# mpt0816/Cilqr

Hardware: AMD Instinct MI355X
Metric: CILQR solves/sec (50-step horizon, batch=65536 per GPU) (higher is better)
Workload: dtype f64

## Files before the change

### cilqr_amd/csrc/cost_reduce.hpp

```cpp
#pragma once
#include "dev_model.hpp"
#include "ref_order.hpp"

namespace cilqr {

CILQR_DEV void reduce_cost(const DeviceState& s, int slot, int cand, double* c5) {
#ifdef CILQR_REF_ORDER
  const int buf = s.cur[slot] ^ cand;
  reforder::total_cost(
      s, slot, [&](int i, double* x) { load_x(s, buf, i, slot, x); }, [&](int i, double* u) { load_u(s, buf, i, slot, u); }, c5);
#else
  (void)cand;
  const int Bc = s.Bcap, K = s.p.K, N = s.p.N;
  double j = 0.0, dx = 0.0, du = 0.0, cc = 0.0, lc = 0.0;
#pragma unroll 8
  for (int i = 0; i < K; ++i) {
    const double2* o = s.part + (size_t)i * kPartPairs * Bc + slot;
    const double2 a = o[0], c = o[(size_t)2 * Bc];
    j += a.x;
    dx += a.y;
    cc += c.x;
    lc += c.y;
  }
#pragma unroll 8
  for (int i = 0; i < N; ++i) {
    const double2 b = s.part[((size_t)i * kPartPairs + 1) * Bc + slot];
    j += b.x;
    du += b.y;
  }
  const double dyn = dx + du;
  c5[0] = j + dyn + cc + lc;
  c5[1] = j; c5[2] = dyn; c5[3] = cc; c5[4] = lc;
#endif
}

#ifdef CILQR_REF_ORDER
CILQR_DEV void spec_total_cost(const DeviceState& s, int slot, int r, int j, double* c5) {
  const size_t cap = (size_t)s.spec_cap;
  reforder::total_cost(
      s, slot,
      [&](int i, double* x) {
        const double2* xb = s.Xs + ((size_t)r * s.p.K + i) * 3 * cap + j;
        const double2 p0 = xb[0], p1 = xb[cap], p2 = xb[2 * cap];
        x[0] = p0.x; x[1] = p0.y; x[2] = p1.x; x[3] = p1.y; x[4] = p2.x; x[5] = p2.y;
      },
      [&](int i, double* u) {
        const double2 q = s.Us[((size_t)r * s.p.N + i) * cap + j];
        u[0] = q.x; u[1] = q.y;
      },
      c5);
}
#endif

}
```

### cilqr_amd/csrc/kernels_quad.hip

```cpp
#include "quad_core.hpp"

namespace cilqr {

#ifndef CILQR_COST_OCC
#define CILQR_COST_OCC 4
#endif
#define CILQR_COST_ATTR __attribute__((amdgpu_waves_per_eu(CILQR_COST_OCC, CILQR_COST_OCC)))
#define CILQR_LAUNCH_BY_DISCS(kernel, grid, block, lds, st, ...)                                            \
  do {                                                                                                     \
    if (s.p.num_of_disc == 5) {                                                                            \
      if (s.exact_ties) hipLaunchKernelGGL((kernel<5, true>), grid, block, lds, st, __VA_ARGS__);          \
      else hipLaunchKernelGGL((kernel<5, false>), grid, block, lds, st, __VA_ARGS__);                      \
    } else {                                                                                               \
      if (s.exact_ties) hipLaunchKernelGGL((kernel<0, true>), grid, block, lds, st, __VA_ARGS__);          \
      else hipLaunchKernelGGL((kernel<0, false>), grid, block, lds, st, __VA_ARGS__);                      \
    }                                                                                                      \
  } while (0)

template <int D, bool EX>
__global__ __launch_bounds__(256) CILQR_COST_ATTR void k_cost_knots(DeviceState s, const int* __restrict__ list,
                                                    const int* __restrict__ n_ptr, int n_max, int cand,
                                                    int skip_done) {
  extern __shared__ double lds[];
#ifdef CILQR_COST_PROFILE
  unsigned long long cp_t = wall_clock64();
  const unsigned long long cp_t0 = cp_t;
#endif
  const int n = n_ptr ? min(*n_ptr, n_max) : active_count(s, n_max);
  if ((int)(blockIdx.x * blockDim.x) >= n) return;
  const double* lanes = stage_lanes(s, lds);
  CP_STAMP(0);
  const int i = blockIdx.y;
// ... 21 lines not shown
#ifdef CILQR_COST_PROFILE
extern "C" void cilqr_debug_cost_profile(unsigned long long* out, int reset) {
  if (out) (void)hipMemcpyFromSymbol(out, HIP_SYMBOL(g_cost_prof), sizeof(g_cost_prof));
  if (reset) { void* p = nullptr; (void)hipGetSymbolAddress(&p, HIP_SYMBOL(g_cost_prof)); (void)hipMemset(p, 0, sizeof(g_cost_prof)); }
}
#endif

template <int D, bool EX>
__global__ __launch_bounds__(256) CILQR_COST_ATTR void k_spec_cost(DeviceState s, const int* __restrict__ list,
                                                   const int* __restrict__ n_ptr, int off, int n_max, int r0) {
  extern __shared__ double lds[];
  const int n = list_count(s, n_ptr, off, n_max);
  if ((int)(blockIdx.x * blockDim.x) >= n) return;
  const double* lanes = stage_lanes(s, lds);
  const int i = blockIdx.y, r = r0 + blockIdx.z;
  const size_t cap = (size_t)s.spec_cap;
  for (int j = blockIdx.x * blockDim.x + threadIdx.x; j < n; j += gridDim.x * blockDim.x) {
    const int slot = list[j];
    if (s.acc_idx[slot] != -1) continue;
    const double2* xb = s.Xs + ((size_t)r * s.p.K + i) * 3 * cap + j;
    const double2 p0 = xb[0], p1 = xb[cap], p2 = xb[2 * cap];
    const double x[6] = {p0.x, p0.y, p1.x, p1.y, p2.x, p2.y};
    double u[2] = {0.0, 0.0};
    if (i < s.p.N) {
      const double2 q = s.Us[((size_t)r * s.p.N + i) * cap + j];
      u[0] = q.x; u[1] = q.y;
    }
    knot_cost<D, EX>(s, lanes, i, slot, x, u, s.parts + ((size_t)r * s.p.K + i) * kPartPairs * cap + j, cap);
  }
}
template <int D, int P, bool EX>
__global__ __launch_bounds__(256) CILQR_COST_ATTR void k_spec_cost_packed(DeviceState s, const int* __restrict__ list,
                                                                          const int* __restrict__ n_ptr, int off, int n_max,
                                                                          int r0, int r_end) {
  extern __shared__ double lds[];
  const int n = list_count(s, n_ptr, off, n_max);
  constexpr int per_block = 256 / P;
  if ((int)(blockIdx.x * per_block) >= n) return;
  const double* lanes = stage_lanes(s, lds);
  const int i = blockIdx.y, r = r0 + (int)(threadIdx.x % P);
  const size_t cap = (size_t)s.spec_cap;
  if (r >= r_end) return;
  for (int j = blockIdx.x * per_block + threadIdx.x / P; j < n; j += gridDim.x * per_block) {
    const int slot = list[j];
    if (s.acc_idx[slot] != -1) continue;
    const double2* xb = s.Xs + ((size_t)r * s.p.K + i) * 3 * cap + j;
    const double2 p0 = xb[0], p1 = xb[cap], p2 = xb[2 * cap];
    const double x[6] = {p0.x, p0.y, p1.x, p1.y, p2.x, p2.y};
    double u[2] = {0.0, 0.0};
    if (i < s.p.N) {
      const double2 q = s.Us[((size_t)r * s.p.N + i) * cap + j];
      u[0] = q.x; u[1] = q.y;
    }
    knot_cost<D, EX>(s, lanes, i, slot, x, u, s.parts + ((size_t)r * s.p.K + i) * kPartPairs * cap + j, cap);
  }
}

void launch_spec_cost(const DeviceState& s, const int* list, const int* n_ptr, int off, int n_max, int n_grid, int r0,
                      int sparse, hipStream_t st) {
  const size_t lds = lane_lds_bytes(s);
  const bool five = s.p.num_of_disc == 5;
  if (!sparse) {
    dim3 g((n_grid + 255) / 256, s.p.K, kNumAlpha - r0);
    CILQR_LAUNCH_BY_DISCS(k_spec_cost, g, dim3(256), lds, st, s, list, n_ptr, off, n_max, r0);
    return;
  }
  for (int a = r0; a < kNumAlpha;) {
    const int left = kNumAlpha - a;
    const int P = left > 4 ? 8 : (left > 2 ? 4 : (left > 1 ? 2 : 1));
    const int e = a + (P < left ? P : left);
    const int per_block = 256 / P;
    dim3 g((n_grid + per_block - 1) / per_block, s.p.K);
#define CILQR_SC1(DD, PP, EE) hipLaunchKernelGGL((k_spec_cost_packed<DD, PP, EE>), g, dim3(256), lds, st, s, list, n_ptr, off, n_max, a, e)
#define CILQR_SC(DD, PP) do { if (s.exact_ties) CILQR_SC1(DD, PP, true); else CILQR_SC1(DD, PP, false); } while (0)
    if (P == 8) { if (five) CILQR_SC(5, 8); else CILQR_SC(0, 8); }
    else if (P == 4) { if (five) CILQR_SC(5, 4); else CILQR_SC(0, 4); }
    else if (P == 2) { if (five) CILQR_SC(5, 2); else CILQR_SC(0, 2); }
    else { if (five) CILQR_SC(5, 1); else CILQR_SC(0, 1); }
#undef CILQR_SC1
#undef CILQR_SC
    a = e;
  }
}

template <int D, int G, bool EX>
__global__ __launch_bounds__(256) CILQR_COST_ATTR void k_round_cost(DeviceState s, int r0, int n_max) {
  extern __shared__ double lds[];
  const int* __restrict__ list = s.pend + (size_t)r0 * s.Bcap;
  const int n = (r0 == 0) ? active_count(s, n_max) : min(s.counters[r0], n_max);
  constexpr int per_block = 256 / G;
  if ((int)(blockIdx.x * per_block) >= n) return;
  const double* lanes = stage_lanes(s, lds);
  const int i = blockIdx.y, r = r0 + (int)(threadIdx.x % G);
  const size_t cap = (size_t)s.spec_cap;
  for (int e = blockIdx.x * per_block + threadIdx.x / G; e < n; e += gridDim.x * per_block) {
    const int j = (r0 == 0) ? e : list[e];
    const int slot = s.act[j];
    if (s.acc_idx[slot] != -1) continue;
    const double2* xb = s.Xs + ((size_t)r * s.p.K + i) * 3 * cap + j;
    const double2 p0 = xb[0], p1 = xb[cap], p2 = xb[2 * cap];
    const double x[6] = {p0.x, p0.y, p1.x, p1.y, p2.x, p2.y};
    double u[2] = {0.0, 0.0};
    if (i < s.p.N) {
      const double2 q = s.Us[((size_t)r * s.p.N + i) * cap + j];
      u[0] = q.x; u[1] = q.y;
    }
    knot_cost<D, EX>(s, lanes, i, slot, x, u, s.parts + ((size_t)r * s.p.K + i) * kPartPairs * cap + j, cap);
  }
}

void launch_round_cost(const DeviceState& s, int r0, int group, int n_max, int n_grid, hipStream_t st) {
  const int per_block = 256 / group;
  dim3 g((n_grid + per_block - 1) / per_block, s.p.K);
  const size_t lds = lane_lds_bytes(s);
  const bool five = s.p.num_of_disc == 5;
#define CILQR_RC1(DD, GG, EE) hipLaunchKernelGGL((k_round_cost<DD, GG, EE>), g, dim3(256), lds, st, s, r0, n_max)
#define CILQR_RC(DD, GG) do { if (s.exact_ties) CILQR_RC1(DD, GG, true); else CILQR_RC1(DD, GG, false); } while (0)
  if (group == 1) { if (five) CILQR_RC(5, 1); else CILQR_RC(0, 1); }
  else if (group == 2) { if (five) CILQR_RC(5, 2); else CILQR_RC(0, 2); }
  else { if (five) CILQR_RC(5, 4); else CILQR_RC(0, 4); }
#undef CILQR_RC
#undef CILQR_RC1
}

__global__ __launch_bounds__(64) void k_reduce_only(DeviceState s, const int* __restrict__ list, int n) {
  const int j = blockIdx.x * blockDim.x + threadIdx.x;
  if (j >= n) return;
  const int slot = list ? list[j] : j;
  double c5[5];
  reduce_cost(s, slot, 0, c5);
#pragma unroll
  for (int c = 0; c < 5; ++c) s.trial[(size_t)c * s.Bcap + slot] = c5[c];
}

void launch_cost_knots(const DeviceState& s, const int* list, const int* n_ptr, int n_max, int n_grid,
                       int cand, int skip_done, hipStream_t st) {
  if (n_grid <= 0) return;
  dim3 g((n_grid + 255) / 256, s.p.K);
  CILQR_LAUNCH_BY_DISCS(k_cost_knots, g, dim3(256), lane_lds_bytes(s), st, s, list, n_ptr, n_max, cand, skip_done);
}

void launch_cost_only(const DeviceState& s, const int* list, int n, int cand, hipStream_t st) {
  if (n == 0) return;
  launch_cost_knots(s, list, nullptr, n, n, cand, 0, st);
  hipLaunchKernelGGL(k_reduce_only, dim3((n + 63) / 64), dim3(64), 0, st, s, list, n);
}

__global__ void k_init_cost_commit(DeviceState s, int n) {
  const int slot = blockIdx.x * blockDim.x + threadIdx.x;
// ... 51 lines not shown
```

### cilqr_amd/csrc/kernels_search.hip

```cpp
#include <cstdio>
#include <cstdlib>

#include "search_core.hpp"

namespace cilqr {

#ifndef CILQR_ROLL_OCC
#define CILQR_ROLL_OCC 0
#endif
#if CILQR_ROLL_OCC > 0
#define CILQR_ROLL_ATTR __attribute__((amdgpu_waves_per_eu(CILQR_ROLL_OCC, CILQR_ROLL_OCC)))
#else
#define CILQR_ROLL_ATTR
#endif
__global__ __launch_bounds__(64) CILQR_ROLL_ATTR void k_forward(DeviceState s, const int* __restrict__ list, int n,
                                                double alpha, int skip_done) {
  const int j = blockIdx.x * blockDim.x + threadIdx.x;
  if (j >= n) return;
  const int slot = list ? list[j] : j;
  if (skip_done && s.acc_idx[slot] != -1) return;
  forward_problem(s, slot, alpha);
}
void launch_forward(const DeviceState& s, const int* list, int n, double alpha, int skip_done,
                    hipStream_t st) {
// ... 43 lines not shown
                                                            const int* __restrict__ n_ptr, int off, int n_max, int r0) {
  const int n = list_count(s, n_ptr, off, n_max);
  constexpr int per_block = 64 / 8;
  const int r = r0 + (threadIdx.x & 7);
  if (r >= kNumAlpha) return;
  for (int j = blockIdx.x * per_block + threadIdx.x / 8; j < n; j += gridDim.x * per_block) {
    const int slot = list[j];
    forward_core(s, slot, kAlpha[r], OutSpec{s, r, j});
  }
}

__global__ __launch_bounds__(64) CILQR_ROLL_ATTR void k_spec_forward(DeviceState s, const int* __restrict__ list,
                                                     const int* __restrict__ n_ptr, int off, int n_max, int r0, int open) {
  const int n = list_count(s, n_ptr, off, n_max);
  const int r = r0 + blockIdx.y;
  for (int j = blockIdx.x * blockDim.x + threadIdx.x; j < n; j += gridDim.x * blockDim.x) {
    const int slot = list[j];
    if (open) {
      if (leaves_before_search(s, slot, r == 0)) {
        if (r == 0) s.acc_idx[slot] = -2;
        continue;
      }
      if (r == 0) s.acc_idx[slot] = -1;
    }
    forward_core(s, slot, kAlpha[r], OutSpec{s, r, j});
  }
}

__global__ __launch_bounds__(64) void k_spec_reduce(DeviceState s, const int* __restrict__ list,
                                                    const int* __restrict__ n_ptr, int off, int n_max, int r0, int open) {
  const int n = list_count(s, n_ptr, off, n_max);
  const int r = r0 + blockIdx.y;
  const size_t cap = (size_t)s.spec_cap;
  const int K = s.p.K, N = s.p.N;
  for (int j = blockIdx.x * blockDim.x + threadIdx.x; j < n; j += gridDim.x * blockDim.x) {
    const int slot = list[j];
    if (open) {
      if (s.acc_idx[slot] != -1) continue;
    }
    double* t = s.spec_tot + (size_t)r * 5 * cap + j;
#ifdef CILQR_REF_ORDER
    double c5[5];
    spec_total_cost(s, slot, r, j, c5);
    t[0] = c5[0];
    t[cap] = c5[1]; t[2 * cap] = c5[2]; t[3 * cap] = c5[3]; t[4 * cap] = c5[4];
    (void)K; (void)N;
#else
    double jj = 0.0, dx = 0.0, du = 0.0, cc = 0.0, lc = 0.0;
    const double2* pb = s.parts + (size_t)r * K * kPartPairs * cap + j;
#pragma unroll 8
    for (int i = 0; i < K; ++i) {
      const double2* o = pb + (size_t)i * kPartPairs * cap;
      const double2 a = o[0], c = o[2 * cap];
      jj += a.x;
      dx += a.y;
      cc += c.x;
      lc += c.y;
    }
#pragma unroll 8
    for (int i = 0; i < N; ++i) {
      const double2 b = pb[((size_t)i * kPartPairs + 1) * cap];
      jj += b.x;
      du += b.y;
    }
    const double dyn = dx + du;
    t[0] = jj + dyn + cc + lc;
    t[cap] = jj; t[2 * cap] = dyn; t[3 * cap] = cc; t[4 * cap] = lc;
#endif
  }
}

__global__ __launch_bounds__(64) void k_spec_pick(DeviceState s, const int* __restrict__ list,
                                                  const int* __restrict__ n_ptr, int off, int n_max, int r0) {
  const int n = list_count(s, n_ptr, off, n_max);
  const size_t cap = (size_t)s.spec_cap;
  const int Bc = s.Bcap;
  for (int j = blockIdx.x * blockDim.x + threadIdx.x; j < n; j += gridDim.x * blockDim.x) {
    const int slot = list[j];
    if (s.acc_idx[slot] != -1) continue;
    const double cost_old = s.cost_old[slot], dV0 = s.dV[slot], dV1 = s.dV[(size_t)Bc + slot];
    int acc = -1, last = kNumAlpha - 1;
    double dcost = 0.0;
    double tot[kNumAlpha];
#pragma unroll
    for (int r = 0; r < kNumAlpha; ++r) tot[r] = (r >= r0) ? s.spec_tot[(size_t)r * 5 * cap + j] : 0.0;
#pragma unroll
    for (int r = 0; r < kNumAlpha; ++r) {
      if (r < r0) continue;
      const double alpha = kAlpha[r];
      dcost = cost_old - tot[r];
      const double expected = -alpha * (dV0 + alpha * dV1);
      const double z = dcost / expected;
      if ((z > 1e-4 && z < 10.0) && dcost > 0.0) {
        acc = r;
        last = r;
        break;
      }
    }
#pragma unroll
    for (int c = 0; c < 5; ++c)
      s.trial[(size_t)c * Bc + slot] = s.spec_tot[((size_t)last * 5 + c) * cap + j];
// ... 31 lines not shown
#ifndef CILQR_FWD_AHEAD
#define CILQR_FWD_AHEAD 1
#endif
template <int P>
__global__ __launch_bounds__(64) __attribute__((amdgpu_waves_per_eu(CILQR_FWD_OCC, CILQR_FWD_OCC)))
void k_multi_forward_packed(DeviceState s, int n, int G) {
  const int t = blockIdx.x * blockDim.x + threadIdx.x;
  const int j = t / P, r = t % P;
  if (j >= active_count(s, n) || r >= G) return;
  const int slot = s.act[j];
  if (leaves_before_search(s, slot, r == 0)) {
    if (r == 0) s.acc_idx[slot] = -2;
    return;
  }
  if (r == 0) s.acc_idx[slot] = -1;
  forward_core<OutSpec, CILQR_FWD_AHEAD>(s, slot, kAlpha[r], OutSpec{s, r, j});
}
template <int G>
__global__ __launch_bounds__(64) void k_multi_forward(DeviceState s, int n) {
  const int j = blockIdx.x * blockDim.x + threadIdx.x;
  if (j >= active_count(s, n)) return;
  const int slot = s.act[j];
  if (leaves_before_search(s, slot, true)) {
    s.acc_idx[slot] = -2;
    return;
  }
  s.acc_idx[slot] = -1;
  forward_multi<G>(s, slot, j);
}

__global__ __launch_bounds__(64) void k_round_pick(DeviceState s, int r0, int G, int n_max, int last) {
  const int* __restrict__ list = s.pend + (size_t)r0 * s.Bcap;
  const int n = (r0 == 0) ? active_count(s, n_max) : min(s.counters[r0], n_max);
  const size_t cap = (size_t)s.spec_cap;
  const int K = s.p.K, N = s.p.N;
  for (int e = blockIdx.x * blockDim.x + threadIdx.x; e < n; e += gridDim.x * blockDim.x) {
    const int j = (r0 == 0) ? e : list[e];
    const int slot = s.act[j];
    if (s.acc_idx[slot] != -1) continue;
    const double cost_old = s.cost_old[slot], dV0 = s.dV[slot], dV1 = s.dV[(size_t)s.Bcap + slot];
    bool accepted = false;
    for (int r = r0; r < r0 + G && !accepted; ++r) {
#ifdef CILQR_REF_ORDER
      double c5[5];
      spec_total_cost(s, slot, r, j, c5);
      (void)K; (void)N; (void)cap;
#else
      double jj = 0.0, dx = 0.0, du = 0.0, cc = 0.0, lc = 0.0;
      const double2* pb = s.parts + (size_t)r * K * kPartPairs * cap + j;
#pragma unroll 8
      for (int i = 0; i < K; ++i) {
        const double2* o = pb + (size_t)i * kPartPairs * cap;
        const double2 a = o[0], c = o[2 * cap];
        jj += a.x;
        dx += a.y;
        cc += c.x;
        lc += c.y;
      }
#pragma unroll 8
      for (int i = 0; i < N; ++i) {
        const double2 b = pb[((size_t)i * kPartPairs + 1) * cap];
        jj += b.x;
        du += b.y;
      }
      const double dyn = dx + du;
      const double c5[5] = {jj + dyn + cc + lc, jj, dyn, cc, lc};
#endif
      const double alpha = kAlpha[r];
      const double dcost = cost_old - c5[0];
      const double expected = -alpha * (dV0 + alpha * dV1);
      const double z = dcost / expected;
#pragma unroll
      for (int c = 0; c < 5; ++c) s.trial[(size_t)c * s.Bcap + slot] = c5[c];
      if ((z > 1e-4 && z < 10.0) && dcost > 0.0) {
        s.acc_idx[slot] = r;
        s.dcost[slot] = dcost;
        s.cur[slot] ^= 1;
        accepted = true;
      }
    }
    if (!accepted && r0 + G < kNumAlpha) {
      const int pos = atomicAdd(&s.counters[r0 + G], 1);
      s.pend[(size_t)(r0 + G) * s.Bcap + pos] = last ? slot : j;
    }
  }
}

constexpr int kCopyKnots = 4;
__global__ __launch_bounds__(256) void k_multi_copy(DeviceState s, int n_max, int G) {
  const int n = active_count(s, n_max);
  const int i0 = blockIdx.y * kCopyKnots;
  const size_t cap = (size_t)s.spec_cap;
  const int K = s.p.K, N = s.p.N, Bc = s.Bcap;
  for (int j = blockIdx.x * blockDim.x + threadIdx.x; j < n; j += gridDim.x * blockDim.x) {
    const int slot = s.act[j];
    const int acc = s.acc_idx[slot];
    if (acc < 0 || acc >= G) continue;
    const int nb = s.cur[slot];
#pragma unroll
    for (int d = 0; d < kCopyKnots; ++d) {
// ... 8 lines not shown
    }
  }
}

static int spec_entries(const DeviceState& s, int n_steps_sizes) {
  static const int forced = [] {
    const char* e = std::getenv("CILQR_SPEC_PASS_ENTRIES");
    return e ? std::atoi(e) : 0;
  }();
  if (s.spec_rows >= kNumAlpha) return s.Bcap;
  const long long cells = (long long)s.spec_rows * s.Bcap;
  int E = (int)(cells / n_steps_sizes);
  if (E >= 64) E = E / 64 * 64;
  if (E > s.Bcap) E = s.Bcap;
  if (forced > 0 && forced < E) E = forced;
  return E;
}
static DeviceState spec_view(const DeviceState& s, int row0, int stride) {
  DeviceState v = s;
  if (s.spec_rows >= kNumAlpha) return v;
  const size_t K = (size_t)s.p.K, N = (size_t)s.p.N;
  if (row0 < 0 || stride <= 0 || (size_t)(kNumAlpha - row0) * (size_t)stride > (size_t)s.spec_rows * (size_t)s.Bcap) {
    std::fprintf(stderr, "cilqr: candidate view [%d..10] x %d does not fit %d x %d cells\n", row0, stride, s.spec_rows, s.Bcap);
    std::abort();
  }
  v.spec_cap = stride;
  v.Xs = reinterpret_cast<double2*>(reinterpret_cast<uintptr_t>(s.Xs) - (uintptr_t)row0 * K * 3 * (size_t)stride * sizeof(double2));
  v.Us = reinterpret_cast<double2*>(reinterpret_cast<uintptr_t>(s.Us) - (uintptr_t)row0 * N * (size_t)stride * sizeof(double2));
  v.parts = reinterpret_cast<double2*>(reinterpret_cast<uintptr_t>(s.parts) - (uintptr_t)row0 * K * kPartPairs * (size_t)stride * sizeof(double2));
  return v;
}
int spec_open_capacity(const DeviceState& s) { return spec_entries(s, kNumAlpha); }

static void launch_spec(const DeviceState& s, const int* list, const int* n_ptr, int off, int n_max, int n_grid, int r0,
                        int open, hipStream_t st) {
  const int na = kNumAlpha - r0;
  const int* lp = list + off;
  const int sparse = (!open && na <= 8) ? 1 : 0;
  if (sparse)
    hipLaunchKernelGGL(k_spec_forward_packed, dim3((n_grid + 7) / 8), dim3(64), 0, st, s, lp, n_ptr, off, n_max, r0);
  else
    hipLaunchKernelGGL(k_spec_forward, dim3((n_grid + 63) / 64, na), dim3(64), 0, st, s, lp, n_ptr, off, n_max, r0, open);
  launch_spec_cost(s, lp, n_ptr, off, n_max, n_grid, r0, sparse, st);
  hipLaunchKernelGGL(k_spec_reduce, dim3((n_grid + 63) / 64, na), dim3(64), 0, st, s, lp, n_ptr, off, n_max, r0, open);
  hipLaunchKernelGGL(k_spec_pick, dim3((n_grid + 63) / 64), dim3(64), 0, st, s, lp, n_ptr, off, n_max, r0);
  hipLaunchKernelGGL(k_spec_copy, dim3((n_grid + 255) / 256, s.p.K), dim3(256), 0, st, s, lp, n_ptr, off, n_max, r0);
}
static void launch_spec_remainder(const DeviceState& s, int R, int n_act, hipStream_t st) {
  const int E = spec_entries(s, kNumAlpha - R);
  const DeviceState v = spec_view(s, R, E);
  for (int off = 0; off < n_act; off += E) {
    const int n_max = (n_act - off < E) ? n_act - off : E;
    const int want = (off == 0) ? (n_act + 3) / 4 : (n_max + 15) / 16;
    const int n_grid = want < n_max ? (want > 0 ? want : 1) : n_max;
    launch_spec(v, s.pend + (size_t)R * s.Bcap, s.counters + R, off, n_max, n_grid, R, 0, st);
  }
}

void launch_linesearch(const DeviceState& s, int n_act, int spec_threshold, int seq_rounds, int round_group,
                       hipStream_t st) {
  if (n_act == 0) return;
  if (n_act <= spec_threshold && n_act <= spec_open_capacity(s)) {
    launch_spec(spec_view(s, 0, spec_open_capacity(s)), s.act, nullptr, 0, n_act, n_act, 0, 1, st);
    return;
  }
  const int R = seq_rounds < 1 ? 1 : (seq_rounds > kNumAlpha ? kNumAlpha : seq_rounds);
  if (R <= kMaxPreRolled && R <= s.spec_rows) {
    const dim3 gf((n_act + 63) / 64), bf(64);
    if (R <= 4) {
      if (R <= 2) hipLaunchKernelGGL(k_multi_forward_packed<2>, dim3((n_act * 2 + 63) / 64), bf, 0, st, s, n_act, R);
      else hipLaunchKernelGGL(k_multi_forward_packed<4>, dim3((n_act * 4 + 63) / 64), bf, 0, st, s, n_act, R);
    }
    else if (R == 5) hipLaunchKernelGGL(k_multi_forward<5>, gf, bf, 0, st, s, n_act);
    else hipLaunchKernelGGL(k_multi_forward<6>, gf, bf, 0, st, s, n_act);
    for (int r0 = 0; r0 < R;) {
      const int G = (round_group >= 4 && R - r0 >= 4) ? 4 : ((round_group >= 2 && R - r0 >= 2) ? 2 : 1);
      const int shrink = (r0 == 0) ? 1 : ((r0 == 1 || G > 1) ? 2 : 8);
      const int n_grid = (n_act + shrink - 1) / shrink;
      launch_round_cost(s, r0, G, n_act, n_grid, st);
      hipLaunchKernelGGL(k_round_pick, dim3((n_act + 63) / 64), dim3(64), 0, st, s, r0, G, n_act, (r0 + G == R) ? 1 : 0);
      r0 += G;
    }
    hipLaunchKernelGGL(k_multi_copy, dim3((n_act + 255) / 256, (s.p.K + kCopyKnots - 1) / kCopyKnots), dim3(256), 0, st, s, n_act, R);
    if (R < kNumAlpha) launch_spec_remainder(s, R, n_act, st);
    return;
  }
  hipLaunchKernelGGL(k_search_open, dim3((n_act + 63) / 64), dim3(64), 0, st, s, n_act);
  for (int r = 0; r < R; ++r) {
    const int shrink = (r == 0) ? 1 : (r == 1 ? 2 : 8);
    const int n_grid = (n_act + shrink - 1) / shrink;
    launch_cost_knots(s, (r == 0) ? (const int*)s.act : (const int*)(s.pend + (size_t)r * s.Bcap),
                      (r == 0) ? (const int*)nullptr : (const int*)(s.counters + r), n_act, n_grid, 1, 1, st);
    hipLaunchKernelGGL(k_search_round, dim3((n_act + 63) / 64), dim3(64), 0, st, s, r, n_act,
                       (r + 1 < R || R == kNumAlpha) ? 1 : 0);
  }
  if (R < kNumAlpha) launch_spec_remainder(s, R, n_act, st);
}

__global__ void k_init_counters(DeviceState s, int first_n) {
  if (threadIdx.x < 64) s.counters[threadIdx.x] = (threadIdx.x == kCntActive) ? first_n : 0;
}
void launch_init_counters(const DeviceState& s, int first_n, hipStream_t st) {
  hipLaunchKernelGGL(k_init_counters, dim3(1), dim3(64), 0, st, s, first_n);
}

CILQR_DEV void update_epilogue(const DeviceState& s) {
  __shared__ int last;
  __syncthreads();
  if (threadIdx.x == 0) {
    __threadfence();
    last = (atomicAdd(&s.counters[kCntTicket], 1) == (int)gridDim.x - 1) ? 1 : 0;
  }
  __syncthreads();
  if (last && threadIdx.x == 0) {
    const int total = atomicAdd(s.n_next, 0);
    *s.h_count_dev = total;
    *s.n_clear = 0;
    s.counters[kCntTicket] = 0;
#pragma unroll
    for (int r = 0; r <= kNumAlpha; ++r) s.counters[r] = 0;
    __threadfence_system();
  }
}

CILQR_DEV void update_problem(const DeviceState& s, int j) {
  const int slot = s.act[j];
  if (!update_state(s, s, slot)) {
    const int pos = atomicAdd(s.n_next, 1);
    s.act_next[pos] = slot;
    if (s.posn) s.posn[slot] = pos;
  }
}
__global__ __launch_bounds__(256) void k_update(DeviceState s, int n) {
// ... 12 lines not shown
```

### cilqr_amd/csrc/search_core.hpp

```cpp
#pragma once
#include "cost_reduce.hpp"

namespace cilqr {

static __device__ const double kAlpha[kNumAlpha] = {1.0000, 0.5012, 0.2512, 0.1259, 0.0631, 0.0316,
                                             0.0158, 0.0079, 0.0040, 0.0020, 0.0010};


struct OutSlot {
  const DeviceState& s;
  int nb, slot;
  CILQR_DEV void x(int i, const double* v) const { store_x(s, nb, i, slot, v); }
  CILQR_DEV void u(int i, const double* v) const { store_u(s, nb, i, slot, v); }
};
struct OutSpec {
  const DeviceState& s;
  int r, j;
  CILQR_DEV void x(int i, const double* v) const {
    const size_t cap = (size_t)s.spec_cap;
    double2* b = s.Xs + ((size_t)r * s.p.K + i) * 3 * cap + j;
    b[0] = make_double2(v[0], v[1]);
    b[cap] = make_double2(v[2], v[3]);
    b[2 * cap] = make_double2(v[4], v[5]);
  }
  CILQR_DEV void u(int i, const double* v) const {
    s.Us[((size_t)r * s.p.N + i) * (size_t)s.spec_cap + j] = make_double2(v[0], v[1]);
  }
};

template <bool InLds>
struct OutSpecSolo {
  double2* xs;
  double2* us;
  CILQR_DEV OutSpecSolo(const DeviceState& s, int r) : xs(s.Xs + (size_t)r * s.p.K * 3), us(s.Us + (size_t)r * s.p.N) {
    assume_lds<InLds>(xs);
    assume_lds<InLds>(us);
  }
  CILQR_DEV void x(int i, const double* v) const {
    double2* b = xs + (size_t)i * 3;
// ... 215 lines not shown
```

### cilqr_amd/csrc/solver.hip

```cpp
#include <hip/hip_runtime.h>

#include <dlfcn.h>
#include <pthread.h>

#include <chrono>
#include <cmath>
#include <condition_variable>
#include <cstdio>
#include <mutex>
#include <thread>
#include <cstdlib>
#include <cstring>
#include <memory>
#include <new>
#include <vector>

#include "build_id.h"
#include "solver_priv.hpp"

using namespace cilqr;

void cilqr_comm_release(cilqr_solver* h);

thread_local char g_last_hip_error[256] = "";
// ... 484 lines not shown
  d.Pcap = Bc;
  auto alloc_moved = [&](DeviceState& t, size_t cap) -> int {
#define ALLOCM(field, count) HIP_TRY(dev_alloc(h, &t.field, (size_t)(count)))
    ALLOCM(X, 2 * K * 3 * cap);
    ALLOCM(U, 2 * N * cap);
    ALLOCM(cur, cap);
    ALLOCM(goals, K * 3 * cap);
    ALLOCM(cor, K * cmax * 3 * cap);
    ALLOCM(ccnt, K * cap);
    ALLOCM(lambda, cap); ALLOCM(dlambda, cap); ALLOCM(cost_old, cap); ALLOCM(dcost, cap);
    ALLOCM(upd, cap); ALLOCM(acc_idx, cap); ALLOCM(emit, cap); ALLOCM(pid, cap); ALLOCM(done_now, cap);
    ALLOCM(act, cap); ALLOCM(act_next, cap); ALLOCM(posn, cap);
#undef ALLOCM
    return CILQR_OK;
  };
  auto alloc_scratch = [&](DeviceState& t, size_t cap) -> int {
#define ALLOCS(field, count) HIP_TRY(dev_alloc(h, &t.field, (size_t)(count)))
    ALLOCS(lin, N * kLinPairs * cap);
    ALLOCS(term, (size_t)kTermPairs * cap);
    ALLOCS(gains, N * kGainPairs * cap);
    ALLOCS(dV, 2 * cap);
    ALLOCS(gnorm, cap);
    ALLOCS(part, K * kPartPairs * cap);
    ALLOCS(trial, 5 * cap);
    t.spec_cap = (int)cap;
    t.spec_rows = (cap >= 32768) ? 4 : kNumAlpha;
    if (const char* e = std::getenv("CILQR_SPEC_ROWS")) t.spec_rows = std::min(kNumAlpha, std::max(4, std::atoi(e)));
    ALLOCS(Xs, (size_t)t.spec_rows * K * 3 * cap);
    ALLOCS(Us, (size_t)t.spec_rows * N * cap);
    ALLOCS(parts, (size_t)t.spec_rows * K * kPartPairs * cap);
    ALLOCS(spec_tot, (size_t)kNumAlpha * 5 * cap);
    ALLOCS(pend, (size_t)(kNumAlpha + 1) * cap);
    ALLOCS(counters, 64);
#undef ALLOCS
    return CILQR_OK;
  };
  if (const int rc = alloc_moved(d, B)) return rc;
  if (const int rc = alloc_scratch(d, B)) return rc;
  HIP_TRY(dev_alloc(h, &d.coarse0, 2 * B));
  HIP_TRY(dev_alloc(h, &d.cstation, K * B));
  h->twin = d;
  if (const int rc = alloc_moved(h->twin, B)) return rc;
  size_t fin_want = 8192;
  if (const char* fe = std::getenv("CILQR_FIN_CAP")) fin_want = (size_t)std::max(64, std::atoi(fe)) / 64 * 64;
  h->fin_cap = (int)std::min<size_t>(B, fin_want);
  h->fin_threshold = h->fin_cap;
  h->fin = d;
  h->fin.Bcap = h->fin_cap;
  if (const int rc = alloc_moved(h->fin, (size_t)h->fin_cap)) return rc;
  if (const int rc = alloc_scratch(h->fin, (size_t)h->fin_cap)) return rc;
  h->fin_twin = h->fin;
  if (const int rc = alloc_moved(h->fin_twin, (size_t)h->fin_cap)) return rc;
  for (cilqr_job_set& js : h->sets) {
    HIP_TRY(dev_alloc(h, &js.hist, (size_t)(cfg->max_iter + 1) * 5 * B));
    HIP_TRY(dev_alloc(h, &js.iter, B));
    HIP_TRY(dev_alloc(h, &js.status, B));
    HIP_TRY(dev_alloc(h, &js.n_cost, B));
    HIP_TRY(dev_alloc(h, &js.n_iter_trajs, B));
    HIP_TRY(dev_alloc(h, &js.atrace, (size_t)cfg->max_iter * B));
    HIP_TRY(dev_alloc(h, &js.lanes, (size_t)2 * max_lane_segments * kLaneFields));
    HIP_TRY(dev_alloc(h, &js.lgrid, (size_t)2 * kGridMaxCells * kGridCellBytes));
    HIP_TRY(dev_alloc(h, &js.lanes_raw, (size_t)2 * max_lane_segments * 7));
    HIP_TRY(dev_alloc(h, &js.tail_iter_dev, 4));
    HIP_TRY(js.h_count.alloc((size_t)(cfg->max_iter + 64) * sizeof(int), hipHostMallocMapped));
    HIP_TRY(hipHostGetDevicePointer(reinterpret_cast<void**>(&js.h_count_dev), js.h_count.get(), 0));
    HIP_TRY(js.handoff.create());
// ... 1098 lines not shown
```

### cilqr_amd/csrc/state.hpp

```cpp
#pragma once

#include <hip/hip_runtime.h>
#include <stdint.h>

namespace cilqr {

constexpr int kNX = 6;
constexpr int kNU = 2;
constexpr int kLinPairs = 17;
constexpr int kTermPairs = 9;
constexpr int kGainPairs = 7;
constexpr int kPartPairs = 3;
constexpr int kNumAlpha = 11;
constexpr int kMaxDiscs = 16;
constexpr int kLaneFields = 11;
constexpr int kGridCellBytes = 16;
#ifndef CILQR_GRID_CELLS_LOG2
#define CILQR_GRID_CELLS_LOG2 16
#endif
constexpr int kGridMaxCells = 1 << CILQR_GRID_CELLS_LOG2;
constexpr int kGridFullScan = 255;

constexpr int kRowA = 0, kRowLx = 6, kRowLu = 9, kRowH = 10, kRowLuu = 16;
constexpr int kDenseDoublesPerStep = 110;
// ... 55 lines not shown
  double* dV;
  double* gnorm;
  double2* part;
  double* trial;
  double* hist;

  int* pid;
  int* done_now;

  double* lambda;
  double* dlambda;
  double* cost_old;
  double* dcost;
  int* iter;
  int* status;
  int* n_cost;
  int* upd;
  int* acc_idx;
  int* n_iter_trajs;
  int* emit;
  signed char* atrace;

  int spec_cap;
  int spec_rows;
  double2* Xs;
  double2* Us;
  double2* parts;
  double* spec_tot;

  int* act;
  int* act_next;
  int* pend;
  int* counters;
  const int* n_dev;
  int* n_next;
  int* n_clear;
  int* h_count_dev;
};
constexpr int kCntActive = 32;
constexpr int kCntTicket = 40;

struct ProblemView {
  const double* start;
  const double* coarse;
  const double* station;
  const double* corridor;
  const int* ccount;
  int cmax_in;
};

void launch_load(const DeviceState& s, int B, const ProblemView& in, const double* lanes_raw,
                 hipStream_t st);
void launch_build_lane_grid(const DeviceState& s, hipStream_t st);
void launch_nearest_lane(const DeviceState& s, int n, const double* xy, int* left, int* right, int use_grid,
                         hipStream_t st);
void launch_init_guess(const DeviceState& s, int B, hipStream_t st);
void launch_init_guess_tracker(const DeviceState& s, const TrackerParams& tp, int B, hipStream_t st);
void launch_set_trajectory(const DeviceState& s, int B, const double* X, const double* U, hipStream_t st);
void launch_cost_only(const DeviceState& s, const int* list, int n, int cand, hipStream_t st);
void launch_cost_knots(const DeviceState& s, const int* list, const int* n_ptr, int n_max, int n_grid,
                       int cand, int skip_done, hipStream_t st);
void launch_spec_cost(const DeviceState& s, const int* list, const int* n_ptr, int off, int n_max, int n_grid, int r0,
                      int sparse, hipStream_t st);
int spec_open_capacity(const DeviceState& s);
void launch_round_cost(const DeviceState& s, int r0, int group, int n_max, int n_grid, hipStream_t st);
void launch_init_cost_commit(const DeviceState& s, int n, hipStream_t st);
void launch_quadratize(const DeviceState& s, const int* list, int n, int only_upd, hipStream_t st);
void launch_backward(const DeviceState& s, const int* list, int n, const double* lambda_override,
                     int team_threshold, int wave_threshold, hipStream_t st, hipEvent_t ev_start = nullptr,
                     hipEvent_t ev_stop = nullptr);
void launch_forward(const DeviceState& s, const int* list, int n, double alpha, int skip_done,
                    hipStream_t st);
void launch_linesearch(const DeviceState& s, int n_act, int spec_threshold, int seq_rounds, int round_group,
                       hipStream_t st);
void launch_init_counters(const DeviceState& s, int first_n, hipStream_t st);
size_t tail_workspace_bytes(const DeviceState& s);
bool tail_supported(const DeviceState& s);
void launch_tail(const DeviceState& s, void* workspace, int n_max, double* traj, double* iter_trajs,
                 int max_iter_trajs, int* max_iter_dev, hipStream_t st);
void launch_update(const DeviceState& s, int n_act, hipStream_t st);
void launch_export_done(const DeviceState& s, int n_act, double* traj, hipStream_t st);
void launch_compact(const DeviceState& src, const DeviceState& dst, int n_max, hipStream_t st);
void launch_export_iter_traj(const DeviceState& s, const int* list, int n, double* iter_trajs,
                             int max_iter_trajs, hipStream_t st);
void launch_export_hist(const DeviceState& s, int B, double* cost_hist, int* n_cost, int* status,
                        int* n_iter, int* n_iter_trajs, signed char* alpha_trace, hipStream_t st);
void launch_export_hist_rows(const DeviceState& s, int B, long long* off, double* rows, hipStream_t st);
constexpr int kCorMaxPts = 320;
struct CorridorParams {
  double max_diff_x, max_diff_y, radius, max_axis_x, max_axis_y;
  int per_edge;
};
void launch_build_corridors(int n, const CorridorParams& cp, const double* knots, const double* points,
                            const int* count, int pmax, double* corridor, int* ccount, int cmax, int* n_failed,
                            double* polygons, hipStream_t st);
struct DpParams;
void launch_dp_place(const DpParams& P, int first, int n_scenes, const double* dyn_poly, const int* dyn_poly_counts,
                     const double* dyn_traj, const int* dyn_traj_counts, double* placed, int* placed_n, hipStream_t st);
// ... 15 lines not shown
```

Before: 2.128 million.

## Fuse line-search cost reduction, pick and copy into cost kernels via last-block epilogue

Adds a per-column-group arrival counter so the last block across the knot dimension of each cost launch runs the total-cost reduction, Armijo acceptance test, pending-list append and trajectory copy. This removes the separate round_pick/multi_copy and spec_reduce/pick/copy launches in the round and sparse speculative paths. It adds atomics, fences and serialized epilogue work on the last-arriving block, plus an abort guard if the grid exceeds the counter array. An env var keeps the old unfused path.

```diff
diff --git a/cilqr_amd/csrc/cost_reduce.hpp b/cilqr_amd/csrc/cost_reduce.hpp
--- a/cilqr_amd/csrc/cost_reduce.hpp
+++ b/cilqr_amd/csrc/cost_reduce.hpp
@@ -52,4 +52,137 @@
 }
 #endif
 
+static __device__ const double kAlpha[kNumAlpha] = {1.0000, 0.5012, 0.2512, 0.1259, 0.0631, 0.0316,
+                                             0.0158, 0.0079, 0.0040, 0.0020, 0.0010};
+
+CILQR_DEV void arena_total_cost(const DeviceState& s, int slot, int r, int j, double* c5) {
+#ifdef CILQR_REF_ORDER
+  spec_total_cost(s, slot, r, j, c5);
+#else
+  (void)slot;
+  const size_t cap = (size_t)s.spec_cap;
+  const int K = s.p.K, N = s.p.N;
+  double jj = 0.0, dx = 0.0, du = 0.0, cc = 0.0, lc = 0.0;
+  const double2* pb = s.parts + (size_t)r * K * kPartPairs * cap + j;
+#pragma unroll 8
+  for (int i = 0; i < K; ++i) {
+    const double2* o = pb + (size_t)i * kPartPairs * cap;
+    const double2 a = o[0], c = o[2 * cap];
+    jj += a.x;
+    dx += a.y;
+    cc += c.x;
+    lc += c.y;
+  }
+#pragma unroll 8
+  for (int i = 0; i < N; ++i) {
+    const double2 b = pb[((size_t)i * kPartPairs + 1) * cap];
+    jj += b.x;
+    du += b.y;
+  }
+  const double dyn = dx + du;
+  c5[0] = jj + dyn + cc + lc;
+  c5[1] = jj; c5[2] = dyn; c5[3] = cc; c5[4] = lc;
+#endif
 }
+
+CILQR_DEV bool group_arrive_last(int* counter, int arrivals, int* flag) {
+  asm volatile("s_waitcnt vmcnt(0)" ::: "memory");
+  __syncthreads();
+  if (threadIdx.x == 0) {
+    __builtin_amdgcn_fence(__ATOMIC_RELEASE, "agent");
+    asm volatile("s_waitcnt vmcnt(0)" ::: "memory");
+    const int ticket = __hip_atomic_fetch_add(counter, 1, __ATOMIC_RELAXED, __HIP_MEMORY_SCOPE_AGENT);
+    const int last = (ticket == arrivals - 1) ? 1 : 0;
+    if (last) {
+      __hip_atomic_store(counter, 0, __ATOMIC_RELAXED, __HIP_MEMORY_SCOPE_AGENT);
+      __builtin_amdgcn_fence(__ATOMIC_ACQUIRE, "agent");
+      asm volatile("s_waitcnt vmcnt(0)" ::: "memory");
+    }
+    *flag = last;
+  }
+  __syncthreads();
+  return *flag != 0;
+}
+
+template <int G>
+CILQR_DEV void group_finish(const DeviceState& s, int r0, int r_end, int n, int grp, int ngrp, const int* positions,
+                            const int* slots, int append, int4* rec) {
+  constexpr int per_block = 256 / G;
+  constexpr int kCopyKnots = 2;
+  const size_t cap = (size_t)s.spec_cap;
+  const int K = s.p.K, N = s.p.N, Bc = s.Bcap;
+  const int q = (int)threadIdx.x / G, g = (int)threadIdx.x % G, r = r0 + g;
+  for (int e0 = grp * per_block; e0 < n; e0 += ngrp * per_block) {
+    const int e = e0 + q;
+    int j = 0, slot = 0, live = 0, cur0 = 0;
+    if (e < n) {
+      j = positions ? positions[e] : e;
+      slot = slots ? slots[e] : s.act[j];
+      if (g == 0) {
+        live = (s.acc_idx[slot] == -1) ? 1 : 0;
+        cur0 = s.cur[slot];
+      }
+    }
+    if constexpr (G > 1) live = __shfl(live, 0, G);
+    double c5[5] = {0.0, 0.0, 0.0, 0.0, 0.0};
+    double dcost = 0.0;
+    int pass = 0;
+    if (live && r < r_end) {
+      arena_total_cost(s, slot, r, j, c5);
+      const double alpha = kAlpha[r];
+      const double dV0 = s.dV[slot], dV1 = s.dV[(size_t)Bc + slot];
+      dcost = s.cost_old[slot] - c5[0];
+      const double expected = -alpha * (dV0 + alpha * dV1);
+      const double z = dcost / expected;
+      pass = ((z > 1e-4 && z < 10.0) && dcost > 0.0) ? 1 : 0;
+    }
+    int win = pass ? 0 : -1;
+    if constexpr (G > 1) {
+      win = -1;
+#pragma unroll
+      for (int k = G - 1; k >= 0; --k)
+        if (__shfl(pass, k, G)) win = k;
+    }
+    const int sel = (win < 0) ? r_end - r0 - 1 : win;
+    double dsel = dcost;
+    if constexpr (G > 1) dsel = __shfl(dcost, sel, G);
+    if (live && g == sel) {
+#pragma unroll
+      for (int c = 0; c < 5; ++c) s.trial[(size_t)c * Bc + slot] = c5[c];
+    }
+    int acc = -1;
+    if (live && g == 0) {
+      if (win >= 0) {
+        acc = r0 + win;
+        s.acc_idx[slot] = acc;
+        s.dcost[slot] = dsel;
+        s.cur[slot] = cur0 ^ 1;
+      } else if (append && r0 + G < kNumAlpha) {
+        const int pos = atomicAdd(&s.counters[r0 + G], 1);
+        s.pend[(size_t)(r0 + G) * Bc + pos] = (append == 2) ? slot : j;
+      }
+    }
+    if (g == 0) rec[q] = make_int4(j, slot, acc, cur0 ^ 1);
+    __syncthreads();
+    for (int w = threadIdx.x; w < per_block * ((K + kCopyKnots - 1) / kCopyKnots); w += 256) {
+      const int4 a = rec[w % per_block];
+      if (a.z < 0) continue;
+      const int i0 = (w / per_block) * kCopyKnots;
+#pragma unroll
+      for (int d = 0; d < kCopyKnots; ++d) {
+        const int i = i0 + d;
+        if (i >= K) break;
+        const double2* xb = s.Xs + ((size_t)a.z * K + i) * 3 * cap + a.x;
+        double2* o = s.X + ((size_t)a.w * K + i) * 3 * Bc + a.y;
+        o[0] = xb[0];
+        o[(size_t)Bc] = xb[cap];
+        o[(size_t)2 * Bc] = xb[2 * cap];
+        if (i < N) s.U[((size_t)a.w * N + i) * Bc + a.y] = s.Us[((size_t)a.z * N + i) * cap + a.x];
+      }
+    }
+    __syncthreads();
+  }
+}
+constexpr size_t kRoundEpilogueLds = 16 + 256 * sizeof(int4);
+
+}
diff --git a/cilqr_amd/csrc/kernels_quad.hip b/cilqr_amd/csrc/kernels_quad.hip
--- a/cilqr_amd/csrc/kernels_quad.hip
+++ b/cilqr_amd/csrc/kernels_quad.hip
@@ -1,3 +1,7 @@
+#include <algorithm>
+#include <cstdio>
+#include <cstdlib>
+
 #include "quad_core.hpp"
 
 namespace cilqr {
@@ -85,7 +89,7 @@
 template <int D, int P, bool EX>
 __global__ __launch_bounds__(256) CILQR_COST_ATTR void k_spec_cost_packed(DeviceState s, const int* __restrict__ list,
                                                                           const int* __restrict__ n_ptr, int off, int n_max,
-                                                                          int r0, int r_end) {
+                                                                          int r0, int r_end, int finish) {
   extern __shared__ double lds[];
   const int n = list_count(s, n_ptr, off, n_max);
   constexpr int per_block = 256 / P;
@@ -93,38 +97,47 @@
   const double* lanes = stage_lanes(s, lds);
   const int i = blockIdx.y, r = r0 + (int)(threadIdx.x % P);
   const size_t cap = (size_t)s.spec_cap;
-  if (r >= r_end) return;
-  for (int j = blockIdx.x * per_block + threadIdx.x / P; j < n; j += gridDim.x * per_block) {
-    const int slot = list[j];
-    if (s.acc_idx[slot] != -1) continue;
-    const double2* xb = s.Xs + ((size_t)r * s.p.K + i) * 3 * cap + j;
-    const double2 p0 = xb[0], p1 = xb[cap], p2 = xb[2 * cap];
-    const double x[6] = {p0.x, p0.y, p1.x, p1.y, p2.x, p2.y};
-    double u[2] = {0.0, 0.0};
-    if (i < s.p.N) {
-      const double2 q = s.Us[((size_t)r * s.p.N + i) * cap + j];
-      u[0] = q.x; u[1] = q.y;
-    }
-    knot_cost<D, EX>(s, lanes, i, slot, x, u, s.parts + ((size_t)r * s.p.K + i) * kPartPairs * cap + j, cap);
-  }
+  if (r < r_end) {
+    for (int j = blockIdx.x * per_block + threadIdx.x / P; j < n; j += gridDim.x * per_block) {
+      const int slot = list[j];
+      if (s.acc_idx[slot] != -1) continue;
+      const double2* xb = s.Xs + ((size_t)r * s.p.K + i) * 3 * cap + j;
+      const double2 p0 = xb[0], p1 = xb[cap], p2 = xb[2 * cap];
+      const double x[6] = {p0.x, p0.y, p1.x, p1.y, p2.x, p2.y};
+      double u[2] = {0.0, 0.0};
+      if (i < s.p.N) {
+        const double2 q = s.Us[((size_t)r * s.p.N + i) * cap + j];
+        u[0] = q.x; u[1] = q.y;
+      }
+      knot_cost<D, EX>(s, lanes, i, slot, x, u, s.parts + ((size_t)r * s.p.K + i) * kPartPairs * cap + j, cap);
+    }
+  }
+  if (finish == 0) return;
+  if (!group_arrive_last(s.grp_cnt + blockIdx.x, (int)gridDim.y, reinterpret_cast<int*>(lds))) return;
+  group_finish<P>(s, r0, r_end, n, (int)blockIdx.x, (int)gridDim.x, nullptr, list, 0, reinterpret_cast<int4*>(lds) + 1);
 }
 
 void launch_spec_cost(const DeviceState& s, const int* list, const int* n_ptr, int off, int n_max, int n_grid, int r0,
-                      int sparse, hipStream_t st) {
-  const size_t lds = lane_lds_bytes(s);
+                      int sparse, int finish, hipStream_t st) {
+  size_t lds = lane_lds_bytes(s);
   const bool five = s.p.num_of_disc == 5;
   if (!sparse) {
     dim3 g((n_grid + 255) / 256, s.p.K, kNumAlpha - r0);
     CILQR_LAUNCH_BY_DISCS(k_spec_cost, g, dim3(256), lds, st, s, list, n_ptr, off, n_max, r0);
     return;
   }
+  if (finish) lds = std::max(lds, kRoundEpilogueLds);
   for (int a = r0; a < kNumAlpha;) {
     const int left = kNumAlpha - a;
     const int P = left > 4 ? 8 : (left > 2 ? 4 : (left > 1 ? 2 : 1));
     const int e = a + (P < left ? P : left);
     const int per_block = 256 / P;
     dim3 g((n_grid + per_block - 1) / per_block, s.p.K);
-#define CILQR_SC1(DD, PP, EE) hipLaunchKernelGGL((k_spec_cost_packed<DD, PP, EE>), g, dim3(256), lds, st, s, list, n_ptr, off, n_max, a, e)
+    if (finish && (e != kNumAlpha || a != r0 || (int)g.x > s.Bcap / 64 + 1)) {
+      std::fprintf(stderr, "cilqr: a speculative pass cannot finish in its cost launch (%d..%d of %d.., %u groups)\n", a, e, r0, g.x);
+      std::abort();
+    }
+#define CILQR_SC1(DD, PP, EE) hipLaunchKernelGGL((k_spec_cost_packed<DD, PP, EE>), g, dim3(256), lds, st, s, list, n_ptr, off, n_max, a, e, finish)
 #define CILQR_SC(DD, PP) do { if (s.exact_ties) CILQR_SC1(DD, PP, true); else CILQR_SC1(DD, PP, false); } while (0)
     if (P == 8) { if (five) CILQR_SC(5, 8); else CILQR_SC(0, 8); }
     else if (P == 4) { if (five) CILQR_SC(5, 4); else CILQR_SC(0, 4); }
@@ -137,37 +150,47 @@
 }
 
 template <int D, int G, bool EX>
-__global__ __launch_bounds__(256) CILQR_COST_ATTR void k_round_cost(DeviceState s, int r0, int n_max) {
+__global__ __launch_bounds__(256) CILQR_COST_ATTR void k_round_cost(DeviceState s, int r0, int n_max, int finish) {
   extern __shared__ double lds[];
   const int* __restrict__ list = s.pend + (size_t)r0 * s.Bcap;
   const int n = (r0 == 0) ? active_count(s, n_max) : min(s.counters[r0], n_max);
   constexpr int per_block = 256 / G;
-  if ((int)(blockIdx.x * per_block) >= n) return;
+  const int grp = blockIdx.x, ngrp = gridDim.x;
+  if (grp * per_block >= n) return;
   const double* lanes = stage_lanes(s, lds);
   const int i = blockIdx.y, r = r0 + (int)(threadIdx.x % G);
   const size_t cap = (size_t)s.spec_cap;
-  for (int e = blockIdx.x * per_block + threadIdx.x / G; e < n; e += gridDim.x * per_block) {
+  for (int e = grp * per_block + threadIdx.x / G; e < n; e += ngrp * per_block) {
     const int j = (r0 == 0) ? e : list[e];
     const int slot = s.act[j];
-    if (s.acc_idx[slot] != -1) continue;
-    const double2* xb = s.Xs + ((size_t)r * s.p.K + i) * 3 * cap + j;
-    const double2 p0 = xb[0], p1 = xb[cap], p2 = xb[2 * cap];
-    const double x[6] = {p0.x, p0.y, p1.x, p1.y, p2.x, p2.y};
-    double u[2] = {0.0, 0.0};
-    if (i < s.p.N) {
-      const double2 q = s.Us[((size_t)r * s.p.N + i) * cap + j];
-      u[0] = q.x; u[1] = q.y;
-    }
-    knot_cost<D, EX>(s, lanes, i, slot, x, u, s.parts + ((size_t)r * s.p.K + i) * kPartPairs * cap + j, cap);
-  }
-}
-
-void launch_round_cost(const DeviceState& s, int r0, int group, int n_max, int n_grid, hipStream_t st) {
+    if (s.acc_idx[slot] == -1) {
+      const double2* xb = s.Xs + ((size_t)r * s.p.K + i) * 3 * cap + j;
+      const double2 p0 = xb[0], p1 = xb[cap], p2 = xb[2 * cap];
+      const double x[6] = {p0.x, p0.y, p1.x, p1.y, p2.x, p2.y};
+      double u[2] = {0.0, 0.0};
+      if (i < s.p.N) {
+        const double2 q = s.Us[((size_t)r * s.p.N + i) * cap + j];
+        u[0] = q.x; u[1] = q.y;
+      }
+      knot_cost<D, EX>(s, lanes, i, slot, x, u, s.parts + ((size_t)r * s.p.K + i) * kPartPairs * cap + j, cap);
+    }
+  }
+  if (finish == 0) return;
+  if (!group_arrive_last(s.grp_cnt + grp, s.p.K, reinterpret_cast<int*>(lds))) return;
+  group_finish<G>(s, r0, r0 + G, n, grp, ngrp, (r0 == 0) ? nullptr : (const int*)list, nullptr, finish,
+                  reinterpret_cast<int4*>(lds) + 1);
+}
+
+void launch_round_cost(const DeviceState& s, int r0, int group, int n_max, int n_grid, int finish, hipStream_t st) {
   const int per_block = 256 / group;
   dim3 g((n_grid + per_block - 1) / per_block, s.p.K);
-  const size_t lds = lane_lds_bytes(s);
+  if (finish && (int)g.x > s.Bcap / 64 + 1) {
+    std::fprintf(stderr, "cilqr: %u groups of a line-search round, %d counters\n", g.x, s.Bcap / 64 + 1);
+    std::abort();
+  }
+  const size_t lds = finish ? std::max(lane_lds_bytes(s), kRoundEpilogueLds) : lane_lds_bytes(s);
   const bool five = s.p.num_of_disc == 5;
-#define CILQR_RC1(DD, GG, EE) hipLaunchKernelGGL((k_round_cost<DD, GG, EE>), g, dim3(256), lds, st, s, r0, n_max)
+#define CILQR_RC1(DD, GG, EE) hipLaunchKernelGGL((k_round_cost<DD, GG, EE>), g, dim3(256), lds, st, s, r0, n_max, finish)
 #define CILQR_RC(DD, GG) do { if (s.exact_ties) CILQR_RC1(DD, GG, true); else CILQR_RC1(DD, GG, false); } while (0)
   if (group == 1) { if (five) CILQR_RC(5, 1); else CILQR_RC(0, 1); }
   else if (group == 2) { if (five) CILQR_RC(5, 2); else CILQR_RC(0, 2); }
diff --git a/cilqr_amd/csrc/kernels_search.hip b/cilqr_amd/csrc/kernels_search.hip
--- a/cilqr_amd/csrc/kernels_search.hip
+++ b/cilqr_amd/csrc/kernels_search.hip
@@ -99,41 +99,16 @@
   const int n = list_count(s, n_ptr, off, n_max);
   const int r = r0 + blockIdx.y;
   const size_t cap = (size_t)s.spec_cap;
-  const int K = s.p.K, N = s.p.N;
   for (int j = blockIdx.x * blockDim.x + threadIdx.x; j < n; j += gridDim.x * blockDim.x) {
     const int slot = list[j];
     if (open) {
       if (s.acc_idx[slot] != -1) continue;
     }
     double* t = s.spec_tot + (size_t)r * 5 * cap + j;
-#ifdef CILQR_REF_ORDER
     double c5[5];
-    spec_total_cost(s, slot, r, j, c5);
+    arena_total_cost(s, slot, r, j, c5);
     t[0] = c5[0];
     t[cap] = c5[1]; t[2 * cap] = c5[2]; t[3 * cap] = c5[3]; t[4 * cap] = c5[4];
-    (void)K; (void)N;
-#else
-    double jj = 0.0, dx = 0.0, du = 0.0, cc = 0.0, lc = 0.0;
-    const double2* pb = s.parts + (size_t)r * K * kPartPairs * cap + j;
-#pragma unroll 8
-    for (int i = 0; i < K; ++i) {
-      const double2* o = pb + (size_t)i * kPartPairs * cap;
-      const double2 a = o[0], c = o[2 * cap];
-      jj += a.x;
-      dx += a.y;
-      cc += c.x;
-      lc += c.y;
-    }
-#pragma unroll 8
-    for (int i = 0; i < N; ++i) {
-      const double2 b = pb[((size_t)i * kPartPairs + 1) * cap];
-      jj += b.x;
-      du += b.y;
-    }
-    const double dyn = dx + du;
-    t[0] = jj + dyn + cc + lc;
-    t[cap] = jj; t[2 * cap] = dyn; t[3 * cap] = cc; t[4 * cap] = lc;
-#endif
   }
 }
 
@@ -231,8 +206,6 @@
 __global__ __launch_bounds__(64) void k_round_pick(DeviceState s, int r0, int G, int n_max, int last) {
   const int* __restrict__ list = s.pend + (size_t)r0 * s.Bcap;
   const int n = (r0 == 0) ? active_count(s, n_max) : min(s.counters[r0], n_max);
-  const size_t cap = (size_t)s.spec_cap;
-  const int K = s.p.K, N = s.p.N;
   for (int e = blockIdx.x * blockDim.x + threadIdx.x; e < n; e += gridDim.x * blockDim.x) {
     const int j = (r0 == 0) ? e : list[e];
     const int slot = s.act[j];
@@ -240,31 +213,8 @@
     const double cost_old = s.cost_old[slot], dV0 = s.dV[slot], dV1 = s.dV[(size_t)s.Bcap + slot];
     bool accepted = false;
     for (int r = r0; r < r0 + G && !accepted; ++r) {
-#ifdef CILQR_REF_ORDER
       double c5[5];
-      spec_total_cost(s, slot, r, j, c5);
-      (void)K; (void)N; (void)cap;
-#else
-      double jj = 0.0, dx = 0.0, du = 0.0, cc = 0.0, lc = 0.0;
-      const double2* pb = s.parts + (size_t)r * K * kPartPairs * cap + j;
-#pragma unroll 8
-      for (int i = 0; i < K; ++i) {
-        const double2* o = pb + (size_t)i * kPartPairs * cap;
-        const double2 a = o[0], c = o[2 * cap];
-        jj += a.x;
-        dx += a.y;
-        cc += c.x;
-        lc += c.y;
-      }
-#pragma unroll 8
-      for (int i = 0; i < N; ++i) {
-        const double2 b = pb[((size_t)i * kPartPairs + 1) * cap];
-        jj += b.x;
-        du += b.y;
-      }
-      const double dyn = dx + du;
-      const double c5[5] = {jj + dyn + cc + lc, jj, dyn, cc, lc};
-#endif
+      arena_total_cost(s, slot, r, j, c5);
       const double alpha = kAlpha[r];
       const double dcost = cost_old - c5[0];
       const double expected = -alpha * (dV0 + alpha * dV1);
@@ -339,6 +289,14 @@
 }
 int spec_open_capacity(const DeviceState& s) { return spec_entries(s, kNumAlpha); }
 
+static int ls_unfused() {
+  static const int unfused = [] {
+    const char* e = std::getenv("CILQR_LS_UNFUSED");
+    return e ? std::atoi(e) : 0;
+  }();
+  return unfused;
+}
+
 static void launch_spec(const DeviceState& s, const int* list, const int* n_ptr, int off, int n_max, int n_grid, int r0,
                         int open, hipStream_t st) {
   const int na = kNumAlpha - r0;
@@ -348,7 +306,9 @@
     hipLaunchKernelGGL(k_spec_forward_packed, dim3((n_grid + 7) / 8), dim3(64), 0, st, s, lp, n_ptr, off, n_max, r0);
   else
     hipLaunchKernelGGL(k_spec_forward, dim3((n_grid + 63) / 64, na), dim3(64), 0, st, s, lp, n_ptr, off, n_max, r0, open);
-  launch_spec_cost(s, lp, n_ptr, off, n_max, n_grid, r0, sparse, st);
+  const int finish = (sparse && ls_unfused() == 0) ? 1 : 0;
+  launch_spec_cost(s, lp, n_ptr, off, n_max, n_grid, r0, sparse, finish, st);
+  if (finish) return;
   hipLaunchKernelGGL(k_spec_reduce, dim3((n_grid + 63) / 64, na), dim3(64), 0, st, s, lp, n_ptr, off, n_max, r0, open);
   hipLaunchKernelGGL(k_spec_pick, dim3((n_grid + 63) / 64), dim3(64), 0, st, s, lp, n_ptr, off, n_max, r0);
   hipLaunchKernelGGL(k_spec_copy, dim3((n_grid + 255) / 256, s.p.K), dim3(256), 0, st, s, lp, n_ptr, off, n_max, r0);
@@ -367,6 +327,7 @@
 void launch_linesearch(const DeviceState& s, int n_act, int spec_threshold, int seq_rounds, int round_group,
                        hipStream_t st) {
   if (n_act == 0) return;
+  const bool unfused = ls_unfused() == 1;
   if (n_act <= spec_threshold && n_act <= spec_open_capacity(s)) {
     launch_spec(spec_view(s, 0, spec_open_capacity(s)), s.act, nullptr, 0, n_act, n_act, 0, 1, st);
     return;
@@ -384,11 +345,12 @@
       const int G = (round_group >= 4 && R - r0 >= 4) ? 4 : ((round_group >= 2 && R - r0 >= 2) ? 2 : 1);
       const int shrink = (r0 == 0) ? 1 : ((r0 == 1 || G > 1) ? 2 : 8);
       const int n_grid = (n_act + shrink - 1) / shrink;
-      launch_round_cost(s, r0, G, n_act, n_grid, st);
-      hipLaunchKernelGGL(k_round_pick, dim3((n_act + 63) / 64), dim3(64), 0, st, s, r0, G, n_act, (r0 + G == R) ? 1 : 0);
+      const int last = (r0 + G == R) ? 1 : 0;
+      launch_round_cost(s, r0, G, n_act, n_grid, unfused ? 0 : 1 + last, st);
+      if (unfused) hipLaunchKernelGGL(k_round_pick, dim3((n_act + 63) / 64), dim3(64), 0, st, s, r0, G, n_act, last);
       r0 += G;
     }
-    hipLaunchKernelGGL(k_multi_copy, dim3((n_act + 255) / 256, (s.p.K + kCopyKnots - 1) / kCopyKnots), dim3(256), 0, st, s, n_act, R);
+    if (unfused) hipLaunchKernelGGL(k_multi_copy, dim3((n_act + 255) / 256, (s.p.K + kCopyKnots - 1) / kCopyKnots), dim3(256), 0, st, s, n_act, R);
     if (R < kNumAlpha) launch_spec_remainder(s, R, n_act, st);
     return;
   }
@@ -406,6 +368,7 @@
 
 __global__ void k_init_counters(DeviceState s, int first_n) {
   if (threadIdx.x < 64) s.counters[threadIdx.x] = (threadIdx.x == kCntActive) ? first_n : 0;
+  for (int g = threadIdx.x; g < s.Bcap / 64 + 1; g += blockDim.x) s.grp_cnt[g] = 0;
 }
 void launch_init_counters(const DeviceState& s, int first_n, hipStream_t st) {
   hipLaunchKernelGGL(k_init_counters, dim3(1), dim3(64), 0, st, s, first_n);
diff --git a/cilqr_amd/csrc/search_core.hpp b/cilqr_amd/csrc/search_core.hpp
--- a/cilqr_amd/csrc/search_core.hpp
+++ b/cilqr_amd/csrc/search_core.hpp
@@ -2,9 +2,6 @@
 #include "cost_reduce.hpp"
 
 namespace cilqr {
-
-static __device__ const double kAlpha[kNumAlpha] = {1.0000, 0.5012, 0.2512, 0.1259, 0.0631, 0.0316,
-                                             0.0158, 0.0079, 0.0040, 0.0020, 0.0010};
 
 
 struct OutSlot {
diff --git a/cilqr_amd/csrc/solver.hip b/cilqr_amd/csrc/solver.hip
--- a/cilqr_amd/csrc/solver.hip
+++ b/cilqr_amd/csrc/solver.hip
@@ -540,6 +540,9 @@
     ALLOCS(spec_tot, (size_t)kNumAlpha * 5 * cap);
     ALLOCS(pend, (size_t)(kNumAlpha + 1) * cap);
     ALLOCS(counters, 64);
+    const size_t n_grp = (cap / 64 + 1 + 3) / 4 * 4;
+    ALLOCS(grp_cnt, n_grp);
+    HIP_TRY(hipMemset(t.grp_cnt, 0, n_grp * sizeof(int)));
 #undef ALLOCS
     return CILQR_OK;
   };
diff --git a/cilqr_amd/csrc/state.hpp b/cilqr_amd/csrc/state.hpp
--- a/cilqr_amd/csrc/state.hpp
+++ b/cilqr_amd/csrc/state.hpp
@@ -111,6 +111,7 @@
   int* act_next;
   int* pend;
   int* counters;
+  int* grp_cnt;
   const int* n_dev;
   int* n_next;
   int* n_clear;
@@ -140,9 +141,9 @@
 void launch_cost_knots(const DeviceState& s, const int* list, const int* n_ptr, int n_max, int n_grid,
                        int cand, int skip_done, hipStream_t st);
 void launch_spec_cost(const DeviceState& s, const int* list, const int* n_ptr, int off, int n_max, int n_grid, int r0,
-                      int sparse, hipStream_t st);
+                      int sparse, int finish, hipStream_t st);
 int spec_open_capacity(const DeviceState& s);
-void launch_round_cost(const DeviceState& s, int r0, int group, int n_max, int n_grid, hipStream_t st);
+void launch_round_cost(const DeviceState& s, int r0, int group, int n_max, int n_grid, int finish, hipStream_t st);
 void launch_init_cost_commit(const DeviceState& s, int n, hipStream_t st);
 void launch_quadratize(const DeviceState& s, const int* list, int n, int only_upd, hipStream_t st);
 void launch_backward(const DeviceState& s, const int* list, int n, const double* lambda_override,
```

Measured after the change: 1.350 million. -36.6%, worse.
